# imulki/serenade

Measured on AMD Instinct MI355X. Metric: mel frames/sec converted (UNet ODE + vocoder), 80x1024, higher is better.
Workload: dtype f32

## Files before the change

### include/serenade_hip.h

```cpp
#ifndef SERENADE_HIP_H
#define SERENADE_HIP_H

#include <stdint.h>

#ifdef __cplusplus
extern "C" {
#endif

#define SRN_ABI_VERSION 4
#define SRN_MAX_TAPS 16

enum { SRN_ACT_NONE = 0, SRN_ACT_LEAKY = 1, SRN_ACT_SILU = 2, SRN_ACT_MISH = 3 };
enum { SRN_RES_NONE = 0, SRN_RES_ADD = 1, SRN_RES_AXPY = 2 };
enum {
  SRN_POST_NONE = 0,
  SRN_POST_DIV = 1,
  SRN_POST_TANH = 2,
  SRN_POST_RELU = 3,
  SRN_POST_LEAKY = 4,
  SRN_POST_GELU = 5
};
enum {
  SRN_PREC_FP32 = 0,
  SRN_PREC_BF16X3 = 1,
// ... 69 lines not shown

int srn_resblock_tail(const float* c2, const float* gn_partials, const float* gamma, const float* beta,
                      const int32_t* lens, const float* r, const float* scale, const float* shift, int64_t ld_ss,
                      float* y, int B, int T, int C, int groups, float gn_eps, float ln_eps, int valid_stats,
                      void* stream);

int srn_resblock_tail_ln(const float* c2, const float* gn_partials, const float* gamma, const float* beta,
                         const int32_t* lens, const float* r, const float* scale, const float* shift, int64_t ld_ss,
                         float* y, int B, int T, int C, int groups, float gn_eps, float ln_eps, int valid_stats,
                         const float* ln2_gamma, const float* ln2_beta, float* y2, float ln2_eps, void* stream);

int srn_layernorm(const float* x, const float* gamma, const float* beta, float* y, int64_t rows, int C, float eps,
                  void* stream);

int srn_softmax_rows(float* s, const int32_t* lens, int Z, int n_head, int L, int ld, void* stream);

int srn_sinusoidal_emb(const float* t, float* out, int n, int dim, int ld, float scale, void* stream);

int srn_copy_channels(const float* src, int64_t src_bs, int ld_src, int sc0, float* dst, int64_t dst_bs, int ld_dst,
                      int dc0, int B, int T, int C, void* stream);

int srn_scatter_rows(const float* src, int64_t src_bs, int ld_src, float* dst, int64_t dst_bs, int ld_dst, int dc0,
                     const int32_t* row_off, const int32_t* n_rows, int B, int T, int C, void* stream);

int srn_transpose_ct(const float* src, float* dst, int B, int R, int Cc, int64_t src_bs, int ld_src, int64_t dst_bs,
                     int ld_dst, void* stream);
#define SRN_TR_LIST_MAX 40
typedef struct SrnTransposeList {
  int32_t n;
  int32_t pad_;
// ... 210 lines not shown
```

### serenade_amd/_lib.py

```python
import ctypes
import os
from ctypes import POINTER, c_char_p, c_double, c_float, c_int, c_int32, c_int64, c_void_p

_HERE = os.path.dirname(os.path.abspath(__file__))
LIB_PATH = os.environ.get("SERENADE_AMD_LIB") or os.path.join(_HERE, "libserenade_hip.so")

SRN_MAX_TAPS = 16
ACT_NONE, ACT_LEAKY, ACT_SILU, ACT_MISH = 0, 1, 2, 3
RES_NONE, RES_ADD, RES_AXPY = 0, 1, 2
POST_NONE, POST_DIV, POST_TANH, POST_RELU, POST_LEAKY, POST_GELU = 0, 1, 2, 3, 4, 5
PREC_FP32, PREC_BF16X3, PREC_BF16X6 = 0, 1, 2
ROUTE_AUTO, ROUTE_TILED, ROUTE_HALO, ROUTE_GENERIC, ROUTE_STRIP, ROUTE_FAST_FP32 = 0, 1, 2, 3, 4, 5
FAMILY_GENERIC, FAMILY_F32, FAMILY_FAST, FAMILY_HALO, FAMILY_STRIP = 0, 1, 2, 3, 4
RESUNIT_ROUTE_SHARED = 1
TN_ROUTE_GENERAL = 1


class SrnConvParams(ctypes.Structure):
    _fields_ = [
        ("n_batch", c_int32), ("n_head", c_int32), ("T_in", c_int32), ("T_out", c_int32),
        ("C_in", c_int32), ("C_in0", c_int32), ("C_w", c_int32), ("N", c_int32), ("N_out", c_int32),
        ("n_taps", c_int32), ("tap_off", c_int32 * SRN_MAX_TAPS), ("in_stride", c_int32),
        ("pad_reflect", c_int32), ("w_nmajor", c_int32), ("pro_act", c_int32), ("pro_slope", c_float),
        ("alpha", c_float), ("beta", c_float), ("geglu", c_int32), ("res_mode", c_int32), ("post", c_int32), ("post_div", c_float),
# ... 78 lines not shown
_SIGS = {
    "srn_abi_version": (c_int, []),
    "srn_last_error": (c_char_p, []),
    "srn_conv_gemm": (c_int, [POINTER(SrnConvParams), _P]),
    "srn_conv_gemm_workspace_bytes": (c_int64, [POINTER(SrnConvParams)]),
    "srn_conv_gemm_route": (c_int, [POINTER(SrnConvParams), POINTER(c_int32)]),
    "srn_hifigan_resunit": (c_int, [POINTER(SrnResUnitParams), _P]),
    "srn_gn_mish_apply": (c_int, [_P, _P, _P, _P, _P, c_int64, _P, _P, c_int, c_int, c_int, c_int, c_float, c_int, _P]),
    "srn_resblock_tail": (c_int, [_P, _P, _P, _P, _P, _P, _P, _P, c_int64, _P, c_int, c_int, c_int, c_int,
                                  c_float, c_float, c_int, _P]),
    "srn_resblock_tail_ln": (c_int, [_P, _P, _P, _P, _P, _P, _P, _P, c_int64, _P, c_int, c_int, c_int, c_int,
                                     c_float, c_float, c_int, _P, _P, _P, c_float, _P]),
    "srn_scatter_rows": (c_int, [_P, c_int64, c_int, _P, c_int64, c_int, c_int, _P, _P, c_int, c_int, c_int, _P]),
    "srn_layernorm": (c_int, [_P, _P, _P, _P, c_int64, c_int, c_float, _P]),
    "srn_softmax_rows": (c_int, [_P, _P, c_int, c_int, c_int, c_int, _P]),
    "srn_sinusoidal_emb": (c_int, [_P, _P, c_int, c_int, c_int, c_float, _P]),
    "srn_copy_channels": (c_int, [_P, c_int64, c_int, c_int, _P, c_int64, c_int, c_int, c_int, c_int, c_int, _P]),
    "srn_transpose_ct": (c_int, [_P, _P, c_int, c_int, c_int, c_int64, c_int, c_int64, c_int, _P]),
    "srn_transpose_multi": (c_int, [POINTER(SrnTransposeList), _P]),
    "srn_weight_norm_fwd": (c_int, [_P, _P, _P, _P, _P, c_int, c_int, c_int, _P]),
    "srn_weight_norm_bwd": (c_int, [_P, _P, _P, _P, _P, _P, c_int, c_int, c_int, _P]),
    "srn_renorm": (c_int, [_P, _P, _P, _P, _P, _P, c_int64, c_int, _P]),
    "srn_out_conv_tanh": (c_int, [_P, _P, _P, _P, c_int, c_int, c_int, c_int, c_float, _P]),
    "srn_pd_gather": (c_int, [_P, _P, _P, c_int, c_int, c_int, c_float, c_float, _P]),
    "srn_pad_signal": (c_int, [_P, _P, c_int, c_int, c_int, c_int, c_int, _P]),
    "srn_logmel": (c_int, [_P, _P, _P, c_int64, c_int, c_int, c_int, c_float, c_int, _P]),
    "srn_loudness": (c_int, [_P, _P, _P, _P, c_int, c_int, c_int, c_int, c_float, c_float, c_float, _P]),
    "srn_gru_recur_last": (c_int, [_P, _P, _P, _P, c_int, c_int, c_int, _P]),
    "srn_style_token_attention_kv": (c_int, [_P] * 8 + [c_int] * 5 + [_P]),
    "srn_rowln_fwd": (c_int, [_P, _P, c_int64, _P, c_int64, _P, c_int, c_int, c_int, c_float, _P]),
# ... 79 lines not shown
```

### serenade_amd/csrc/norm_act.hip

```cpp
#include "common.h"
#include "conv_common.h"

namespace {

__device__ __forceinline__ void group_stats(const float* __restrict__ partials, int b, int T, int C, int groups,
                                            float eps, float* s_mean, float* s_rstd, int n_rows) {
  const int gn_mt = (T + 31) / 32;
  const int gn_nt = C / 32;
  const int nt_per_g = (C / groups) / 32;
  const int wave = threadIdx.x >> 6, lane = threadIdx.x & 63;
  const float* base = partials + (int64_t)b * gn_mt * gn_nt * 2;
  const int per_g = gn_mt * nt_per_g;
  for (int g = wave; g < groups; g += 4) {
    double s1 = 0.0, s2 = 0.0;
    for (int e = lane; e < per_g; e += 64) {
      const int mt = e / nt_per_g;
      const int nt = g * nt_per_g + (e - mt * nt_per_g);
      const float2 v = *reinterpret_cast<const float2*>(base + ((int64_t)mt * gn_nt + nt) * 2);
      s1 += (double)v.x;
      s2 += (double)v.y;
    }
    s1 = wave_sum_d(s1);
    s2 = wave_sum_d(s2);
    if (lane == 0) {
      const double cnt = (double)max(n_rows, 1) * (double)(C / groups);
      const double mean = s1 / cnt;
      double var = s2 / cnt - mean * mean;
      if (var < 0.0) var = 0.0;
      s_mean[g] = (float)mean;
      s_rstd[g] = (float)(1.0 / sqrt(var + (double)eps));
    }
  }
  __syncthreads();
}

constexpr int GN_ROWS = 8;
constexpr int SMALL_GRID = 512;
constexpr int GN_PRE = 4;

__global__ __launch_bounds__(256) void gn_mish_apply_kernel(const float* __restrict__ x,
                                                            const float* __restrict__ partials,
                                                            const float* __restrict__ gamma,
                                                            const float* __restrict__ beta,
                                                            const float* __restrict__ time_bias,
                                                            const int32_t* __restrict__ lens, float* __restrict__ y,
                                                            int T, int C, int groups, float eps, int64_t tb_bs,
                                                            int valid_stats, int rows_per_wg) {
  __shared__ float s_mean[64], s_rstd[64];
  const int b = blockIdx.y;
  const int r0 = blockIdx.x * rows_per_wg;
  if (time_bias) time_bias += (int64_t)b * tb_bs;
  const int len = lens ? min(lens[b], T) : T;
  const int c4n = C / 4;
  const int cpg = C / groups;
  const int rows = min(rows_per_wg, T - r0);
// ... 35 lines not shown
  };
#pragma unroll
  for (int k = 0; k < GN_PRE; ++k)
    if ((int)threadIdx.x + 256 * k < total) one(threadIdx.x + 256 * k, pre[k]);
  for (int idx = threadIdx.x + 256 * GN_PRE; idx < total; idx += 256) {
    const int r = idx / c4n;
    float4 v = make_float4(0.f, 0.f, 0.f, 0.f);
    if (r0 + r < len) v = *reinterpret_cast<const float4*>(x + base + (int64_t)r * C + (idx - r * c4n) * 4);
    one(idx, v);
  }
}

constexpr int TAIL_ROWS = 8;
constexpr int MAXV = 4;

__global__ __launch_bounds__(256) void resblock_tail_kernel(
    const float* __restrict__ c2, const float* __restrict__ partials, const float* __restrict__ gamma,
    const float* __restrict__ beta, const int32_t* __restrict__ lens, const float* __restrict__ rres,
    const float* __restrict__ scale, const float* __restrict__ shift, int64_t ld_ss, float* __restrict__ y, int T,
    int C, int groups, float gn_eps, float ln_eps, int valid_stats, const float* __restrict__ ln2_gamma,
    const float* __restrict__ ln2_beta, float* __restrict__ y2, float ln2_eps, int rows_per_wg) {
  __shared__ float s_mean[64], s_rstd[64];
  const int b = blockIdx.y;
  const int r0 = blockIdx.x * rows_per_wg;
  const int len = lens ? min(lens[b], T) : T;
  const int wave = threadIdx.x >> 6, lane = threadIdx.x & 63;
  const int c4n = C / 4;
  const int cpg = C / groups;
  const float inv_c = 1.0f / (float)C;
  const int r_end = min(r0 + rows_per_wg, T);
  float4 xin[MAXV], rin[MAXV];
// ... 88 lines not shown
          const int c = c4 * 4;
          const float4 ga = *reinterpret_cast<const float4*>(ln2_gamma + c);
          const float4 be = *reinterpret_cast<const float4*>(ln2_beta + c);
          float4 o;
          o.x = (v[i].x - mean2) * rstd2 * ga.x + be.x;
          o.y = (v[i].y - mean2) * rstd2 * ga.y + be.y;
          o.z = (v[i].z - mean2) * rstd2 * ga.z + be.z;
          o.w = (v[i].w - mean2) * rstd2 * ga.w + be.w;
          *reinterpret_cast<float4*>(y2 + row + c) = o;
        }
      }
    }
  }
}

__global__ __launch_bounds__(256) void layernorm_kernel(const float* __restrict__ x, const float* __restrict__ gamma,
                                                        const float* __restrict__ beta, float* __restrict__ y,
                                                        int64_t rows, int C, float eps) {
  const int wave = threadIdx.x >> 6, lane = threadIdx.x & 63;
  const int c4n = C / 4;
  const float inv_c = 1.0f / (float)C;
  for (int64_t r = (int64_t)blockIdx.x * 4 + wave; r < rows; r += (int64_t)gridDim.x * 4) {
    const int64_t row = r * C;
    float4 v[MAXV];
    float sum = 0.f;
#pragma unroll
    for (int i = 0; i < MAXV; ++i) {
      const int c4 = lane + 64 * i;
      v[i] = make_float4(0.f, 0.f, 0.f, 0.f);
      if (c4 < c4n) {
        v[i] = *reinterpret_cast<const float4*>(x + row + c4 * 4);
// ... 17 lines not shown
        const int c = c4 * 4;
        const float4 ga = *reinterpret_cast<const float4*>(gamma + c);
        const float4 be = *reinterpret_cast<const float4*>(beta + c);
        float4 o;
        o.x = (v[i].x - mean) * rstd * ga.x + be.x;
        o.y = (v[i].y - mean) * rstd * ga.y + be.y;
        o.z = (v[i].z - mean) * rstd * ga.z + be.z;
        o.w = (v[i].w - mean) * rstd * ga.w + be.w;
        *reinterpret_cast<float4*>(y + row + c) = o;
      }
    }
  }
}

template <int NV>
__global__ __launch_bounds__(256) void softmax_rows_kernel(float* __restrict__ s, const int32_t* __restrict__ lens,
                                                           int64_t n_rows, int n_head, int L, int ld) {
  const int wave = threadIdx.x >> 6, lane = threadIdx.x & 63;
  const int64_t r = (int64_t)blockIdx.x * 4 + wave;
  if (r >= n_rows) return;
  const int z = (int)(r / L);
  int len = L;
  if (lens) len = min(lens[z / n_head], L);
  float* row = s + r * ld;
  const int ld4 = ld / 4;
  float4 v[NV];
  float mx = -INFINITY;
#pragma unroll
  for (int i = 0; i < NV; ++i) {
    const int c4 = lane + 64 * i;
    v[i] = make_float4(-INFINITY, -INFINITY, -INFINITY, -INFINITY);
// ... 19 lines not shown
      sum += (v[i].x + v[i].y) + (v[i].z + v[i].w);
    }
  }
  sum = wave_sum(sum);
#pragma unroll
  for (int i = 0; i < NV; ++i) {
    const int c4 = lane + 64 * i;
    if (c4 < ld4) {
      float4 o;
      o.x = v[i].x / sum;
      o.y = v[i].y / sum;
      o.z = v[i].z / sum;
      o.w = v[i].w / sum;
      *reinterpret_cast<float4*>(row + c4 * 4) = o;
    }
  }
}

__global__ void sinusoidal_emb_kernel(const float* __restrict__ t, float* __restrict__ out, int n, int dim,
                                      int ld, float scale) {
  const int half = dim / 2;
  const int idx = blockIdx.x * blockDim.x + threadIdx.x;
  if (idx >= n * half) return;
  const int i = idx / half, k = idx - i * half;
  const float emb = logf(10000.0f) / (float)(half - 1);
  const float f = expf((float)k * -emb);
  const float arg = scale * t[i] * f;
  out[(int64_t)i * ld + k] = sinf(arg);
  out[(int64_t)i * ld + half + k] = cosf(arg);
}
// ... 140 lines not shown
  float acc = bias[0];
  for (int j = 0; j < K; ++j) {
    const int ti = t + j - (K - 1) / 2;
    if (ti < 0 || ti >= T) continue;
    for (int c = 0; c < C; ++c) {
      float v = xb[(int64_t)ti * C + c];
      v = v > 0.f ? v : v * slope;
      acc = fmaf(v, w[j * C + c], acc);
    }
  }
  y[(int64_t)b * T + t] = tanhf(acc);
}

}

extern "C" int srn_gn_mish_apply(const float* x, const float* gn_partials, const float* gamma, const float* beta,
                                 const float* time_bias, int64_t time_bias_bs, const int32_t* lens, float* y, int B,
                                 int T, int C, int groups, float eps, int valid_stats, void* stream) {
  SRN_CHECK_ARG(x && gn_partials && gamma && beta && y, "gn_mish_apply: null pointer");
  SRN_CHECK_ARG(!valid_stats || lens, "gn_mish_apply: valid_stats needs lens");
  SRN_CHECK_ARG(B > 0 && T > 0 && C > 0 && groups > 0 && groups <= 64 && C % groups == 0 && (C / groups) % 32 == 0,
                "gn_mish_apply: need (C / groups) %% 32 == 0 (C=%d groups=%d)", C, groups);
  const int rows_per_wg = (int64_t)B * ((T + GN_ROWS - 1) / GN_ROWS) < SMALL_GRID ? GN_ROWS / 2 : GN_ROWS;
  dim3 grid((T + rows_per_wg - 1) / rows_per_wg, B);
  hipLaunchKernelGGL(gn_mish_apply_kernel, grid, dim3(256), 0, (hipStream_t)stream, x, gn_partials, gamma, beta,
                     time_bias, lens, y, T, C, groups, eps, time_bias_bs, valid_stats, rows_per_wg);
  SRN_CHECK_LAUNCH();
  return 0;
}

extern "C" int srn_resblock_tail(const float* c2, const float* gn_partials, const float* gamma, const float* beta,
                                 const int32_t* lens, const float* r, const float* scale, const float* shift,
                                 int64_t ld_ss, float* y, int B, int T, int C, int groups, float gn_eps,
                                 float ln_eps, int valid_stats, void* stream) {
  SRN_CHECK_ARG(c2 && gn_partials && gamma && beta && r && scale && shift && y, "resblock_tail: null pointer");
  SRN_CHECK_ARG(!valid_stats || lens, "resblock_tail: valid_stats needs lens");
  SRN_CHECK_ARG(B > 0 && T > 0 && C > 0 && C % 4 == 0 && C <= 256 * MAXV, "resblock_tail: C=%d unsupported", C);
  SRN_CHECK_ARG(groups > 0 && groups <= 64 && C % groups == 0 && (C / groups) % 32 == 0,
                "resblock_tail: need (C / groups) %% 32 == 0");
  const int rows_per_wg = (int64_t)B * ((T + TAIL_ROWS - 1) / TAIL_ROWS) < SMALL_GRID ? TAIL_ROWS / 2 : TAIL_ROWS;
  dim3 grid((T + rows_per_wg - 1) / rows_per_wg, B);
  hipLaunchKernelGGL(resblock_tail_kernel, grid, dim3(256), 0, (hipStream_t)stream, c2, gn_partials, gamma, beta,
                     lens, r, scale, shift, ld_ss, y, T, C, groups, gn_eps, ln_eps, valid_stats, nullptr, nullptr,
                     nullptr, 0.f, rows_per_wg);
  SRN_CHECK_LAUNCH();
  return 0;
}

extern "C" int srn_resblock_tail_ln(const float* c2, const float* gn_partials, const float* gamma, const float* beta,
                                    const int32_t* lens, const float* r, const float* scale, const float* shift,
                                    int64_t ld_ss, float* y, int B, int T, int C, int groups, float gn_eps,
                                    float ln_eps, int valid_stats, const float* ln2_gamma, const float* ln2_beta,
                                    float* y2, float ln2_eps, void* stream) {
  SRN_CHECK_ARG(c2 && gn_partials && gamma && beta && r && scale && shift && y && ln2_gamma && ln2_beta && y2,
                "resblock_tail_ln: null pointer");
  SRN_CHECK_ARG(!valid_stats || lens, "resblock_tail_ln: valid_stats needs lens");
  SRN_CHECK_ARG(B > 0 && T > 0 && C > 0 && C % 4 == 0 && C <= 256 * MAXV, "resblock_tail_ln: C=%d unsupported", C);
  SRN_CHECK_ARG(groups > 0 && groups <= 64 && C % groups == 0 && (C / groups) % 32 == 0,
                "resblock_tail_ln: need (C / groups) %% 32 == 0");
  const int rows_per_wg = (int64_t)B * ((T + TAIL_ROWS - 1) / TAIL_ROWS) < SMALL_GRID ? TAIL_ROWS / 2 : TAIL_ROWS;
  dim3 grid((T + rows_per_wg - 1) / rows_per_wg, B);
  hipLaunchKernelGGL(resblock_tail_kernel, grid, dim3(256), 0, (hipStream_t)stream, c2, gn_partials, gamma, beta,
                     lens, r, scale, shift, ld_ss, y, T, C, groups, gn_eps, ln_eps, valid_stats, ln2_gamma, ln2_beta,
                     y2, ln2_eps, rows_per_wg);
  SRN_CHECK_LAUNCH();
  return 0;
}

extern "C" int srn_layernorm(const float* x, const float* gamma, const float* beta, float* y, int64_t rows, int C,
                             float eps, void* stream) {
  SRN_CHECK_ARG(x && gamma && beta && y, "layernorm: null pointer");
  SRN_CHECK_ARG(rows > 0 && C > 0 && C % 4 == 0 && C <= 256 * MAXV, "layernorm: C=%d unsupported", C);
  int64_t blocks = (rows + 3) / 4;
  if (blocks > 65536) blocks = 65536;
  hipLaunchKernelGGL(layernorm_kernel, dim3((unsigned)blocks), dim3(256), 0, (hipStream_t)stream, x, gamma, beta, y,
                     rows, C, eps);
  SRN_CHECK_LAUNCH();
  return 0;
}

extern "C" int srn_softmax_rows(float* s, const int32_t* lens, int Z, int n_head, int L, int ld, void* stream) {
  SRN_CHECK_ARG(s != nullptr && Z > 0 && n_head > 0 && L > 0 && ld >= L && ld % 4 == 0, "softmax_rows: bad args");
  const int64_t rows = (int64_t)Z * L;
  const unsigned blocks = (unsigned)((rows + 3) / 4);
  const int nv = (ld / 4 + 63) / 64;
  hipStream_t st = (hipStream_t)stream;
  if (nv <= 2) hipLaunchKernelGGL(softmax_rows_kernel<2>, dim3(blocks), dim3(256), 0, st, s, lens, rows, n_head, L, ld);
  else if (nv <= 4) hipLaunchKernelGGL(softmax_rows_kernel<4>, dim3(blocks), dim3(256), 0, st, s, lens, rows, n_head, L, ld);
  else if (nv <= 8) hipLaunchKernelGGL(softmax_rows_kernel<8>, dim3(blocks), dim3(256), 0, st, s, lens, rows, n_head, L, ld);
  else if (nv <= 12) hipLaunchKernelGGL(softmax_rows_kernel<12>, dim3(blocks), dim3(256), 0, st, s, lens, rows, n_head, L, ld);
  else if (nv <= 20) hipLaunchKernelGGL(softmax_rows_kernel<20>, dim3(blocks), dim3(256), 0, st, s, lens, rows, n_head, L, ld);
  else if (nv <= 36) hipLaunchKernelGGL(softmax_rows_kernel<36>, dim3(blocks), dim3(256), 0, st, s, lens, rows, n_head, L, ld);
  else {
    srn_set_error("softmax_rows: L=%d too long (max 9216)", L);
    return -1;
  }
  SRN_CHECK_LAUNCH();
  return 0;
}

extern "C" int srn_sinusoidal_emb(const float* t, float* out, int n, int dim, int ld, float scale, void* stream) {
  SRN_CHECK_ARG(t && out && n > 0 && dim > 2 && dim % 2 == 0 && ld >= dim, "sinusoidal_emb: bad args");
  const int total = n * (dim / 2);
  hipLaunchKernelGGL(sinusoidal_emb_kernel, dim3((total + 255) / 256), dim3(256), 0, (hipStream_t)stream, t, out, n,
                     dim, ld, scale);
  SRN_CHECK_LAUNCH();
  return 0;
}

extern "C" int srn_copy_channels(const float* src, int64_t src_bs, int ld_src, int sc0, float* dst, int64_t dst_bs,
                                 int ld_dst, int dc0, int B, int T, int C, void* stream) {
// ... 120 lines not shown
```

Measured before the change: 61660.

## Make row-wise norm/softmax kernels persistent with double-buffered buffer loads

```diff
diff --git a/include/serenade_hip.h b/include/serenade_hip.h
--- a/include/serenade_hip.h
+++ b/include/serenade_hip.h
@@ -107,6 +107,21 @@
                   void* stream);
 
 int srn_softmax_rows(float* s, const int32_t* lens, int Z, int n_head, int L, int ld, void* stream);
+
+int srn_gn_mish_apply_r4(const float* x, const float* gn_partials, const float* gamma, const float* beta,
+                         const float* time_bias, int64_t time_bias_bs, const int32_t* lens, float* y, int B, int T,
+                         int C, int groups, float eps, int valid_stats, void* stream);
+int srn_resblock_tail_r4(const float* c2, const float* gn_partials, const float* gamma, const float* beta,
+                         const int32_t* lens, const float* r, const float* scale, const float* shift, int64_t ld_ss,
+                         float* y, int B, int T, int C, int groups, float gn_eps, float ln_eps, int valid_stats,
+                         void* stream);
+int srn_resblock_tail_ln_r4(const float* c2, const float* gn_partials, const float* gamma, const float* beta,
+                            const int32_t* lens, const float* r, const float* scale, const float* shift, int64_t ld_ss,
+                            float* y, int B, int T, int C, int groups, float gn_eps, float ln_eps, int valid_stats,
+                            const float* ln2_gamma, const float* ln2_beta, float* y2, float ln2_eps, void* stream);
+int srn_layernorm_r4(const float* x, const float* gamma, const float* beta, float* y, int64_t rows, int C, float eps,
+                     void* stream);
+int srn_softmax_rows_r4(float* s, const int32_t* lens, int Z, int n_head, int L, int ld, void* stream);
 
 int srn_sinusoidal_emb(const float* t, float* out, int n, int dim, int ld, float scale, void* stream);
 
diff --git a/serenade_amd/_lib.py b/serenade_amd/_lib.py
--- a/serenade_amd/_lib.py
+++ b/serenade_amd/_lib.py
@@ -116,6 +116,13 @@
     "srn_scatter_rows": (c_int, [_P, c_int64, c_int, _P, c_int64, c_int, c_int, _P, _P, c_int, c_int, c_int, _P]),
     "srn_layernorm": (c_int, [_P, _P, _P, _P, c_int64, c_int, c_float, _P]),
     "srn_softmax_rows": (c_int, [_P, _P, c_int, c_int, c_int, c_int, _P]),
+    "srn_gn_mish_apply_r4": (c_int, [_P, _P, _P, _P, _P, c_int64, _P, _P, c_int, c_int, c_int, c_int, c_float, c_int, _P]),
+    "srn_resblock_tail_r4": (c_int, [_P, _P, _P, _P, _P, _P, _P, _P, c_int64, _P, c_int, c_int, c_int, c_int,
+                                     c_float, c_float, c_int, _P]),
+    "srn_resblock_tail_ln_r4": (c_int, [_P, _P, _P, _P, _P, _P, _P, _P, c_int64, _P, c_int, c_int, c_int, c_int,
+                                        c_float, c_float, c_int, _P, _P, _P, c_float, _P]),
+    "srn_layernorm_r4": (c_int, [_P, _P, _P, _P, c_int64, c_int, c_float, _P]),
+    "srn_softmax_rows_r4": (c_int, [_P, _P, c_int, c_int, c_int, c_int, _P]),
     "srn_sinusoidal_emb": (c_int, [_P, _P, c_int, c_int, c_int, c_float, _P]),
     "srn_copy_channels": (c_int, [_P, c_int64, c_int, c_int, _P, c_int64, c_int, c_int, c_int, c_int, c_int, _P]),
     "srn_transpose_ct": (c_int, [_P, _P, c_int, c_int, c_int, c_int64, c_int, c_int64, c_int, _P]),
diff --git a/serenade_amd/csrc/norm_act.hip b/serenade_amd/csrc/norm_act.hip
--- a/serenade_amd/csrc/norm_act.hip
+++ b/serenade_amd/csrc/norm_act.hip
@@ -1,5 +1,7 @@
 #include "common.h"
 #include "conv_common.h"
+
+#include <algorithm>
 
 namespace {
 
@@ -38,7 +40,7 @@
 constexpr int SMALL_GRID = 512;
 constexpr int GN_PRE = 4;
 
-__global__ __launch_bounds__(256) void gn_mish_apply_kernel(const float* __restrict__ x,
+__global__ __launch_bounds__(256) void gn_mish_apply_r4_kernel(const float* __restrict__ x,
                                                             const float* __restrict__ partials,
                                                             const float* __restrict__ gamma,
                                                             const float* __restrict__ beta,
@@ -104,7 +106,7 @@
 constexpr int TAIL_ROWS = 8;
 constexpr int MAXV = 4;
 
-__global__ __launch_bounds__(256) void resblock_tail_kernel(
+__global__ __launch_bounds__(256) void resblock_tail_r4_kernel(
     const float* __restrict__ c2, const float* __restrict__ partials, const float* __restrict__ gamma,
     const float* __restrict__ beta, const int32_t* __restrict__ lens, const float* __restrict__ rres,
     const float* __restrict__ scale, const float* __restrict__ shift, int64_t ld_ss, float* __restrict__ y, int T,
@@ -223,7 +225,7 @@
   }
 }
 
-__global__ __launch_bounds__(256) void layernorm_kernel(const float* __restrict__ x, const float* __restrict__ gamma,
+__global__ __launch_bounds__(256) void layernorm_r4_kernel(const float* __restrict__ x, const float* __restrict__ gamma,
                                                         const float* __restrict__ beta, float* __restrict__ y,
                                                         int64_t rows, int C, float eps) {
   const int wave = threadIdx.x >> 6, lane = threadIdx.x & 63;
@@ -271,7 +273,7 @@
 }
 
 template <int NV>
-__global__ __launch_bounds__(256) void softmax_rows_kernel(float* __restrict__ s, const int32_t* __restrict__ lens,
+__global__ __launch_bounds__(256) void softmax_rows_r4_kernel(float* __restrict__ s, const int32_t* __restrict__ lens,
                                                            int64_t n_rows, int n_head, int L, int ld) {
   const int wave = threadIdx.x >> 6, lane = threadIdx.x & 63;
   const int64_t r = (int64_t)blockIdx.x * 4 + wave;
@@ -321,6 +323,399 @@
       o.w = v[i].w / sum;
       *reinterpret_cast<float4*>(row + c4 * 4) = o;
     }
+  }
+}
+
+constexpr int ROW_WGS_PER_CU = 4;
+
+typedef unsigned rw_u32x4 __attribute__((ext_vector_type(4)));
+
+__device__ __forceinline__ __amdgpu_buffer_rsrc_t row_rsrc(const float* row, int bytes) {
+  return __builtin_amdgcn_make_buffer_rsrc(const_cast<float*>(row), 0, bytes, 0x00020000);
+}
+__device__ __forceinline__ float4 row_ld(__amdgpu_buffer_rsrc_t rs, int off) {
+  return __builtin_bit_cast(float4, __builtin_amdgcn_raw_buffer_load_b128(rs, off, 0, 0));
+}
+__device__ __forceinline__ void row_st(const float4 v, __amdgpu_buffer_rsrc_t rs, int off) {
+  __builtin_amdgcn_raw_buffer_store_b128(__builtin_bit_cast(rw_u32x4, v), rs, off, 0, 0);
+}
+
+__device__ __forceinline__ void gn_worker_rows(int T, int rpw, int& t_begin, int& t_end) {
+  t_begin = blockIdx.x * 4 * rpw;
+  t_end = min(t_begin + 4 * rpw, T);
+}
+
+template <int NV>
+__global__ __launch_bounds__(256) void gn_mish_apply_kernel(const float* __restrict__ x,
+                                                            const float* __restrict__ partials,
+                                                            const float* __restrict__ gamma,
+                                                            const float* __restrict__ beta,
+                                                            const float* __restrict__ time_bias,
+                                                            const int32_t* __restrict__ lens, float* __restrict__ y,
+                                                            int T, int C, int groups, float eps, int64_t tb_bs,
+                                                            int valid_stats, int rpw) {
+  __shared__ float s_mean[64], s_rstd[64];
+  const int b = blockIdx.y;
+  const int wave = __builtin_amdgcn_readfirstlane(threadIdx.x >> 6), lane = threadIdx.x & 63;
+  int t_begin, t_end;
+  gn_worker_rows(T, rpw, t_begin, t_end);
+  const int len = lens ? min(lens[b], T) : T;
+  const int c4n = C / 4;
+  const int cpg = C / groups;
+  const float* xb = x + (int64_t)b * T * C;
+  float* yb = y + (int64_t)b * T * C;
+  auto fetch = [&](float4 (&v)[NV], const int t) {
+    if (t >= len) return;
+    const __amdgpu_buffer_rsrc_t rs = row_rsrc(xb + (int64_t)t * C, C * 4);
+#pragma unroll
+    for (int i = 0; i < NV; ++i)
+      if (lane + 64 * i < c4n) v[i] = row_ld(rs, (lane + 64 * i) * 16);
+  };
+  float4 va[NV], vb[NV];
+  int t = t_begin + wave;
+  if (t < t_end) fetch(va, t);
+  group_stats(partials, b, T, C, groups, eps, s_mean, s_rstd, valid_stats ? len : T);
+  float4 ga[NV], be[NV], tb[NV];
+  float m[NV], rsd[NV];
+#pragma unroll
+  for (int i = 0; i < NV; ++i) {
+    const int c = (lane + 64 * i) * 4;
+    ga[i] = be[i] = tb[i] = make_float4(0.f, 0.f, 0.f, 0.f);
+    m[i] = rsd[i] = 0.f;
+    if (lane + 64 * i < c4n) {
+      ga[i] = *reinterpret_cast<const float4*>(gamma + c);
+      be[i] = *reinterpret_cast<const float4*>(beta + c);
+      if (time_bias) tb[i] = *reinterpret_cast<const float4*>(time_bias + (int64_t)b * tb_bs + c);
+      m[i] = s_mean[c / cpg];
+      rsd[i] = s_rstd[c / cpg];
+    }
+  }
+  auto finish = [&](const float4 (&v)[NV], const int t) {
+    const __amdgpu_buffer_rsrc_t rs = row_rsrc(yb + (int64_t)t * C, C * 4);
+    const bool valid = t < len;
+#pragma unroll
+    for (int i = 0; i < NV; ++i) {
+      if (lane + 64 * i < c4n) {
+        float4 o = make_float4(0.f, 0.f, 0.f, 0.f);
+        if (valid) {
+          o.x = srn_mish((v[i].x - m[i]) * rsd[i] * ga[i].x + be[i].x);
+          o.y = srn_mish((v[i].y - m[i]) * rsd[i] * ga[i].y + be[i].y);
+          o.z = srn_mish((v[i].z - m[i]) * rsd[i] * ga[i].z + be[i].z);
+          o.w = srn_mish((v[i].w - m[i]) * rsd[i] * ga[i].w + be[i].w);
+          if (time_bias) {
+            o.x += tb[i].x;
+            o.y += tb[i].y;
+            o.z += tb[i].z;
+            o.w += tb[i].w;
+          }
+        }
+        row_st(o, rs, (lane + 64 * i) * 16);
+      }
+    }
+  };
+  while (t < t_end) {
+    if (t + 4 < t_end) fetch(vb, t + 4);
+    finish(va, t);
+    t += 4;
+    if (t >= t_end) break;
+    if (t + 4 < t_end) fetch(va, t + 4);
+    finish(vb, t);
+    t += 4;
+  }
+}
+
+template <int NV>
+__global__ __launch_bounds__(256) void resblock_tail_kernel(
+    const float* __restrict__ c2, const float* __restrict__ partials, const float* __restrict__ gamma,
+    const float* __restrict__ beta, const int32_t* __restrict__ lens, const float* __restrict__ rres,
+    const float* __restrict__ scale, const float* __restrict__ shift, int64_t ld_ss, float* __restrict__ y, int T,
+    int C, int groups, float gn_eps, float ln_eps, int valid_stats, const float* __restrict__ ln2_gamma,
+    const float* __restrict__ ln2_beta, float* __restrict__ y2, float ln2_eps, int rpw) {
+  __shared__ float s_mean[64], s_rstd[64];
+  const int b = blockIdx.y;
+  const int wave = __builtin_amdgcn_readfirstlane(threadIdx.x >> 6), lane = threadIdx.x & 63;
+  int t_begin, t_end;
+  gn_worker_rows(T, rpw, t_begin, t_end);
+  const int len = lens ? min(lens[b], T) : T;
+  const int c4n = C / 4;
+  const int cpg = C / groups;
+  const float inv_c = 1.0f / (float)C;
+  const int64_t base = (int64_t)b * T * C;
+  struct Row {
+    float4 x[NV], r[NV];
+  };
+  auto fetch = [&](Row& a, const int t) {
+    const __amdgpu_buffer_rsrc_t rr = row_rsrc(rres + base + (int64_t)t * C, C * 4);
+    const __amdgpu_buffer_rsrc_t rx = row_rsrc(c2 + base + (int64_t)t * C, C * 4);
+#pragma unroll
+    for (int i = 0; i < NV; ++i) {
+      a.x[i] = a.r[i] = make_float4(0.f, 0.f, 0.f, 0.f);
+      if (lane + 64 * i < c4n) {
+        a.r[i] = row_ld(rr, (lane + 64 * i) * 16);
+        if (t < len) a.x[i] = row_ld(rx, (lane + 64 * i) * 16);
+      }
+    }
+  };
+  Row ra, rb;
+  int t = t_begin + wave;
+  if (t < t_end) fetch(ra, t);
+  group_stats(partials, b, T, C, groups, gn_eps, s_mean, s_rstd, valid_stats ? len : T);
+  float4 ga[NV], be[NV], sc[NV], sh[NV], lg[NV], lb[NV];
+  float m[NV], rsd[NV];
+#pragma unroll
+  for (int i = 0; i < NV; ++i) {
+    const int c = (lane + 64 * i) * 4;
+    ga[i] = be[i] = sc[i] = sh[i] = lg[i] = lb[i] = make_float4(0.f, 0.f, 0.f, 0.f);
+    m[i] = rsd[i] = 0.f;
+    if (lane + 64 * i < c4n) {
+      ga[i] = *reinterpret_cast<const float4*>(gamma + c);
+      be[i] = *reinterpret_cast<const float4*>(beta + c);
+      sc[i] = *reinterpret_cast<const float4*>(scale + (int64_t)b * ld_ss + c);
+      sh[i] = *reinterpret_cast<const float4*>(shift + (int64_t)b * ld_ss + c);
+      if (y2 != nullptr) {
+        lg[i] = *reinterpret_cast<const float4*>(ln2_gamma + c);
+        lb[i] = *reinterpret_cast<const float4*>(ln2_beta + c);
+      }
+      m[i] = s_mean[c / cpg];
+      rsd[i] = s_rstd[c / cpg];
+    }
+  }
+  auto finish = [&](const Row& a, const int t) {
+    const int64_t row = base + (int64_t)t * C;
+    const bool valid = t < len;
+    float4 v[NV];
+    float sum = 0.f;
+#pragma unroll
+    for (int i = 0; i < NV; ++i) {
+      v[i] = make_float4(0.f, 0.f, 0.f, 0.f);
+      if (lane + 64 * i < c4n) {
+        const float4 rr = a.r[i];
+        float4 o = make_float4(0.f, 0.f, 0.f, 0.f);
+        if (valid) {
+          const float4 xx = a.x[i];
+          o.x = srn_mish((xx.x - m[i]) * rsd[i] * ga[i].x + be[i].x);
+          o.y = srn_mish((xx.y - m[i]) * rsd[i] * ga[i].y + be[i].y);
+          o.z = srn_mish((xx.z - m[i]) * rsd[i] * ga[i].z + be[i].z);
+          o.w = srn_mish((xx.w - m[i]) * rsd[i] * ga[i].w + be[i].w);
+        }
+        v[i] = make_float4(o.x + rr.x, o.y + rr.y, o.z + rr.z, o.w + rr.w);
+        sum += (v[i].x + v[i].y) + (v[i].z + v[i].w);
+      }
+    }
+    const float mean = wave_sum(sum) * inv_c;
+    float sq = 0.f;
+#pragma unroll
+    for (int i = 0; i < NV; ++i) {
+      if (lane + 64 * i < c4n) {
+        const float dx = v[i].x - mean, dy = v[i].y - mean, dz = v[i].z - mean, dw = v[i].w - mean;
+        sq += (dx * dx + dy * dy) + (dz * dz + dw * dw);
+      }
+    }
+    const float stdv = sqrtf(wave_sum(sq) * inv_c + ln_eps);
+    const __amdgpu_buffer_rsrc_t ry = row_rsrc(y + row, C * 4);
+#pragma unroll
+    for (int i = 0; i < NV; ++i) {
+      if (lane + 64 * i < c4n) {
+        float4 o;
+        o.x = (v[i].x - mean) / stdv * sc[i].x + sh[i].x;
+        o.y = (v[i].y - mean) / stdv * sc[i].y + sh[i].y;
+        o.z = (v[i].z - mean) / stdv * sc[i].z + sh[i].z;
+        o.w = (v[i].w - mean) / stdv * sc[i].w + sh[i].w;
+        row_st(o, ry, (lane + 64 * i) * 16);
+        v[i] = o;
+      }
+    }
+    if (y2 != nullptr) {
+      float sum2 = 0.f;
+#pragma unroll
+      for (int i = 0; i < NV; ++i)
+        if (lane + 64 * i < c4n) sum2 += (v[i].x + v[i].y) + (v[i].z + v[i].w);
+      const float mean2 = wave_sum(sum2) * inv_c;
+      float sq2 = 0.f;
+#pragma unroll
+      for (int i = 0; i < NV; ++i) {
+        if (lane + 64 * i < c4n) {
+          const float dx = v[i].x - mean2, dy = v[i].y - mean2, dz = v[i].z - mean2, dw = v[i].w - mean2;
+          sq2 += (dx * dx + dy * dy) + (dz * dz + dw * dw);
+        }
+      }
+      const float rstd2 = 1.0f / sqrtf(wave_sum(sq2) * inv_c + ln2_eps);
+      const __amdgpu_buffer_rsrc_t ry2 = row_rsrc(y2 + row, C * 4);
+#pragma unroll
+      for (int i = 0; i < NV; ++i) {
+        if (lane + 64 * i < c4n) {
+          float4 o;
+          o.x = (v[i].x - mean2) * rstd2 * lg[i].x + lb[i].x;
+          o.y = (v[i].y - mean2) * rstd2 * lg[i].y + lb[i].y;
+          o.z = (v[i].z - mean2) * rstd2 * lg[i].z + lb[i].z;
+          o.w = (v[i].w - mean2) * rstd2 * lg[i].w + lb[i].w;
+          row_st(o, ry2, (lane + 64 * i) * 16);
+        }
+      }
+    }
+  };
+  while (t < t_end) {
+    if (t + 4 < t_end) fetch(rb, t + 4);
+    finish(ra, t);
+    t += 4;
+    if (t >= t_end) break;
+    if (t + 4 < t_end) fetch(ra, t + 4);
+    finish(rb, t);
+    t += 4;
+  }
+}
+
+template <int NV>
+__global__ __launch_bounds__(256) void layernorm_kernel(const float* __restrict__ x, const float* __restrict__ gamma,
+                                                        const float* __restrict__ beta, float* __restrict__ y,
+                                                        int64_t rows, int C, float eps) {
+  const int lane = threadIdx.x & 63;
+  const int64_t stride = (int64_t)gridDim.x * 4;
+  int64_t r = (int64_t)blockIdx.x * 4 + __builtin_amdgcn_readfirstlane(threadIdx.x >> 6);
+  if (r >= rows) return;
+  const int c4n = C / 4;
+  const float inv_c = 1.0f / (float)C;
+  auto fetch = [&](float4 (&v)[NV], const int64_t rr) {
+    const __amdgpu_buffer_rsrc_t rs = row_rsrc(x + rr * C, C * 4);
+#pragma unroll
+    for (int i = 0; i < NV; ++i)
+      if (lane + 64 * i < c4n) v[i] = row_ld(rs, (lane + 64 * i) * 16);
+  };
+  float4 va[NV], vb[NV];
+  fetch(va, r);
+  float4 ga[NV], be[NV];
+#pragma unroll
+  for (int i = 0; i < NV; ++i) {
+    ga[i] = be[i] = make_float4(0.f, 0.f, 0.f, 0.f);
+    if (lane + 64 * i < c4n) {
+      ga[i] = *reinterpret_cast<const float4*>(gamma + (lane + 64 * i) * 4);
+      be[i] = *reinterpret_cast<const float4*>(beta + (lane + 64 * i) * 4);
+    }
+  }
+  auto finish = [&](const float4 (&v)[NV], const int64_t rr) {
+    float sum = 0.f;
+#pragma unroll
+    for (int i = 0; i < NV; ++i)
+      if (lane + 64 * i < c4n) sum += (v[i].x + v[i].y) + (v[i].z + v[i].w);
+    const float mean = wave_sum(sum) * inv_c;
+    float sq = 0.f;
+#pragma unroll
+    for (int i = 0; i < NV; ++i) {
+      if (lane + 64 * i < c4n) {
+        const float dx = v[i].x - mean, dy = v[i].y - mean, dz = v[i].z - mean, dw = v[i].w - mean;
+        sq += (dx * dx + dy * dy) + (dz * dz + dw * dw);
+      }
+    }
+    const float rstd = 1.0f / sqrtf(wave_sum(sq) * inv_c + eps);
+    const __amdgpu_buffer_rsrc_t rs = row_rsrc(y + rr * C, C * 4);
+#pragma unroll
+    for (int i = 0; i < NV; ++i) {
+      if (lane + 64 * i < c4n) {
+        float4 o;
+        o.x = (v[i].x - mean) * rstd * ga[i].x + be[i].x;
+        o.y = (v[i].y - mean) * rstd * ga[i].y + be[i].y;
+        o.z = (v[i].z - mean) * rstd * ga[i].z + be[i].z;
+        o.w = (v[i].w - mean) * rstd * ga[i].w + be[i].w;
+        row_st(o, rs, (lane + 64 * i) * 16);
+      }
+    }
+  };
+  for (;;) {
+    if (r + stride < rows) fetch(vb, r + stride);
+    finish(va, r);
+    r += stride;
+    if (r >= rows) return;
+    if (r + stride < rows) fetch(va, r + stride);
+    finish(vb, r);
+    r += stride;
+    if (r >= rows) return;
+  }
+}
+
+template <int NV>
+struct SmRow {
+  float4 v[NV];
+  int len;
+};
+
+template <int NV, bool AHEAD>
+__global__ __launch_bounds__(256) void softmax_rows_kernel(float* __restrict__ s, const int32_t* __restrict__ lens,
+                                                           int n_rows, int n_head, int L, int ld) {
+  const int lane = threadIdx.x & 63;
+  const int stride = gridDim.x * 4;
+  int r = blockIdx.x * 4 + __builtin_amdgcn_readfirstlane(threadIdx.x >> 6);
+  if (r >= n_rows) return;
+  const int ld4 = ld / 4;
+  auto fetch = [&](SmRow<NV>& a, const int rr) {
+    const __amdgpu_buffer_rsrc_t rs = row_rsrc(s + (int64_t)rr * ld, ld * 4);
+#pragma unroll
+    for (int i = 0; i < NV; ++i)
+      if (lane + 64 * i < ld4) a.v[i] = row_ld(rs, (lane + 64 * i) * 16);
+    a.len = lens ? min(lens[rr / L / n_head], L) : L;
+  };
+  auto finish = [&](const SmRow<NV>& a, const int rr) {
+    const int len = a.len;
+    float4 v[NV];
+    float mx = -INFINITY;
+#pragma unroll
+    for (int i = 0; i < NV; ++i) {
+      const int c4 = lane + 64 * i;
+      v[i] = make_float4(-INFINITY, -INFINITY, -INFINITY, -INFINITY);
+      if (c4 < ld4) {
+        const float4 t = a.v[i];
+        const int c = c4 * 4;
+        if (c + 0 < len) v[i].x = t.x;
+        if (c + 1 < len) v[i].y = t.y;
+        if (c + 2 < len) v[i].z = t.z;
+        if (c + 3 < len) v[i].w = t.w;
+        mx = fmaxf(mx, fmaxf(fmaxf(v[i].x, v[i].y), fmaxf(v[i].z, v[i].w)));
+      }
+    }
+    mx = wave_max(mx);
+    float sum = 0.f;
+#pragma unroll
+    for (int i = 0; i < NV; ++i) {
+      if (lane + 64 * i < ld4) {
+        v[i].x = expf(v[i].x - mx);
+        v[i].y = expf(v[i].y - mx);
+        v[i].z = expf(v[i].z - mx);
+        v[i].w = expf(v[i].w - mx);
+        sum += (v[i].x + v[i].y) + (v[i].z + v[i].w);
+      }
+    }
+    sum = wave_sum(sum);
+    const __amdgpu_buffer_rsrc_t rs = row_rsrc(s + (int64_t)rr * ld, ld * 4);
+#pragma unroll
+    for (int i = 0; i < NV; ++i) {
+      const int c4 = lane + 64 * i;
+      if (c4 < ld4) {
+        float4 o;
+        o.x = v[i].x / sum;
+        o.y = v[i].y / sum;
+        o.z = v[i].z / sum;
+        o.w = v[i].w / sum;
+        row_st(o, rs, c4 * 16);
+      }
+    }
+  };
+  SmRow<NV> ra, rb;
+  fetch(ra, r);
+  for (;;) {
+    if (!AHEAD) {
+      finish(ra, r);
+      r += stride;
+      if (r >= n_rows) return;
+      fetch(ra, r);
+      continue;
+    }
+    if (r + stride < n_rows) fetch(rb, r + stride);
+    finish(ra, r);
+    r += stride;
+    if (r >= n_rows) return;
+    if (r + stride < n_rows) fetch(ra, r + stride);
+    finish(rb, r);
+    r += stride;
+    if (r >= n_rows) return;
   }
 }
 
@@ -491,7 +886,7 @@
 
 }
 
-extern "C" int srn_gn_mish_apply(const float* x, const float* gn_partials, const float* gamma, const float* beta,
+extern "C" int srn_gn_mish_apply_r4(const float* x, const float* gn_partials, const float* gamma, const float* beta,
                                  const float* time_bias, int64_t time_bias_bs, const int32_t* lens, float* y, int B,
                                  int T, int C, int groups, float eps, int valid_stats, void* stream) {
   SRN_CHECK_ARG(x && gn_partials && gamma && beta && y, "gn_mish_apply: null pointer");
@@ -500,13 +895,13 @@
                 "gn_mish_apply: need (C / groups) %% 32 == 0 (C=%d groups=%d)", C, groups);
   const int rows_per_wg = (int64_t)B * ((T + GN_ROWS - 1) / GN_ROWS) < SMALL_GRID ? GN_ROWS / 2 : GN_ROWS;
   dim3 grid((T + rows_per_wg - 1) / rows_per_wg, B);
-  hipLaunchKernelGGL(gn_mish_apply_kernel, grid, dim3(256), 0, (hipStream_t)stream, x, gn_partials, gamma, beta,
+  hipLaunchKernelGGL(gn_mish_apply_r4_kernel, grid, dim3(256), 0, (hipStream_t)stream, x, gn_partials, gamma, beta,
                      time_bias, lens, y, T, C, groups, eps, time_bias_bs, valid_stats, rows_per_wg);
   SRN_CHECK_LAUNCH();
   return 0;
 }
 
-extern "C" int srn_resblock_tail(const float* c2, const float* gn_partials, const float* gamma, const float* beta,
+extern "C" int srn_resblock_tail_r4(const float* c2, const float* gn_partials, const float* gamma, const float* beta,
                                  const int32_t* lens, const float* r, const float* scale, const float* shift,
                                  int64_t ld_ss, float* y, int B, int T, int C, int groups, float gn_eps,
                                  float ln_eps, int valid_stats, void* stream) {
@@ -517,14 +912,14 @@
                 "resblock_tail: need (C / groups) %% 32 == 0");
   const int rows_per_wg = (int64_t)B * ((T + TAIL_ROWS - 1) / TAIL_ROWS) < SMALL_GRID ? TAIL_ROWS / 2 : TAIL_ROWS;
   dim3 grid((T + rows_per_wg - 1) / rows_per_wg, B);
-  hipLaunchKernelGGL(resblock_tail_kernel, grid, dim3(256), 0, (hipStream_t)stream, c2, gn_partials, gamma, beta,
+  hipLaunchKernelGGL(resblock_tail_r4_kernel, grid, dim3(256), 0, (hipStream_t)stream, c2, gn_partials, gamma, beta,
                      lens, r, scale, shift, ld_ss, y, T, C, groups, gn_eps, ln_eps, valid_stats, nullptr, nullptr,
                      nullptr, 0.f, rows_per_wg);
   SRN_CHECK_LAUNCH();
   return 0;
 }
 
-extern "C" int srn_resblock_tail_ln(const float* c2, const float* gn_partials, const float* gamma, const float* beta,
+extern "C" int srn_resblock_tail_ln_r4(const float* c2, const float* gn_partials, const float* gamma, const float* beta,
                                     const int32_t* lens, const float* r, const float* scale, const float* shift,
                                     int64_t ld_ss, float* y, int B, int T, int C, int groups, float gn_eps,
                                     float ln_eps, int valid_stats, const float* ln2_gamma, const float* ln2_beta,
@@ -537,41 +932,193 @@
                 "resblock_tail_ln: need (C / groups) %% 32 == 0");
   const int rows_per_wg = (int64_t)B * ((T + TAIL_ROWS - 1) / TAIL_ROWS) < SMALL_GRID ? TAIL_ROWS / 2 : TAIL_ROWS;
   dim3 grid((T + rows_per_wg - 1) / rows_per_wg, B);
-  hipLaunchKernelGGL(resblock_tail_kernel, grid, dim3(256), 0, (hipStream_t)stream, c2, gn_partials, gamma, beta,
+  hipLaunchKernelGGL(resblock_tail_r4_kernel, grid, dim3(256), 0, (hipStream_t)stream, c2, gn_partials, gamma, beta,
                      lens, r, scale, shift, ld_ss, y, T, C, groups, gn_eps, ln_eps, valid_stats, ln2_gamma, ln2_beta,
                      y2, ln2_eps, rows_per_wg);
   SRN_CHECK_LAUNCH();
   return 0;
 }
 
-extern "C" int srn_layernorm(const float* x, const float* gamma, const float* beta, float* y, int64_t rows, int C,
+extern "C" int srn_layernorm_r4(const float* x, const float* gamma, const float* beta, float* y, int64_t rows, int C,
                              float eps, void* stream) {
   SRN_CHECK_ARG(x && gamma && beta && y, "layernorm: null pointer");
   SRN_CHECK_ARG(rows > 0 && C > 0 && C % 4 == 0 && C <= 256 * MAXV, "layernorm: C=%d unsupported", C);
   int64_t blocks = (rows + 3) / 4;
   if (blocks > 65536) blocks = 65536;
-  hipLaunchKernelGGL(layernorm_kernel, dim3((unsigned)blocks), dim3(256), 0, (hipStream_t)stream, x, gamma, beta, y,
+  hipLaunchKernelGGL(layernorm_r4_kernel, dim3((unsigned)blocks), dim3(256), 0, (hipStream_t)stream, x, gamma, beta, y,
                      rows, C, eps);
   SRN_CHECK_LAUNCH();
   return 0;
 }
 
-extern "C" int srn_softmax_rows(float* s, const int32_t* lens, int Z, int n_head, int L, int ld, void* stream) {
+extern "C" int srn_softmax_rows_r4(float* s, const int32_t* lens, int Z, int n_head, int L, int ld, void* stream) {
   SRN_CHECK_ARG(s != nullptr && Z > 0 && n_head > 0 && L > 0 && ld >= L && ld % 4 == 0, "softmax_rows: bad args");
   const int64_t rows = (int64_t)Z * L;
   const unsigned blocks = (unsigned)((rows + 3) / 4);
   const int nv = (ld / 4 + 63) / 64;
   hipStream_t st = (hipStream_t)stream;
-  if (nv <= 2) hipLaunchKernelGGL(softmax_rows_kernel<2>, dim3(blocks), dim3(256), 0, st, s, lens, rows, n_head, L, ld);
-  else if (nv <= 4) hipLaunchKernelGGL(softmax_rows_kernel<4>, dim3(blocks), dim3(256), 0, st, s, lens, rows, n_head, L, ld);
-  else if (nv <= 8) hipLaunchKernelGGL(softmax_rows_kernel<8>, dim3(blocks), dim3(256), 0, st, s, lens, rows, n_head, L, ld);
-  else if (nv <= 12) hipLaunchKernelGGL(softmax_rows_kernel<12>, dim3(blocks), dim3(256), 0, st, s, lens, rows, n_head, L, ld);
-  else if (nv <= 20) hipLaunchKernelGGL(softmax_rows_kernel<20>, dim3(blocks), dim3(256), 0, st, s, lens, rows, n_head, L, ld);
-  else if (nv <= 36) hipLaunchKernelGGL(softmax_rows_kernel<36>, dim3(blocks), dim3(256), 0, st, s, lens, rows, n_head, L, ld);
+  if (nv <= 2) hipLaunchKernelGGL(softmax_rows_r4_kernel<2>, dim3(blocks), dim3(256), 0, st, s, lens, rows, n_head, L, ld);
+  else if (nv <= 4) hipLaunchKernelGGL(softmax_rows_r4_kernel<4>, dim3(blocks), dim3(256), 0, st, s, lens, rows, n_head, L, ld);
+  else if (nv <= 8) hipLaunchKernelGGL(softmax_rows_r4_kernel<8>, dim3(blocks), dim3(256), 0, st, s, lens, rows, n_head, L, ld);
+  else if (nv <= 12) hipLaunchKernelGGL(softmax_rows_r4_kernel<12>, dim3(blocks), dim3(256), 0, st, s, lens, rows, n_head, L, ld);
+  else if (nv <= 20) hipLaunchKernelGGL(softmax_rows_r4_kernel<20>, dim3(blocks), dim3(256), 0, st, s, lens, rows, n_head, L, ld);
+  else if (nv <= 36) hipLaunchKernelGGL(softmax_rows_r4_kernel<36>, dim3(blocks), dim3(256), 0, st, s, lens, rows, n_head, L, ld);
   else {
     srn_set_error("softmax_rows: L=%d too long (max 9216)", L);
     return -1;
   }
+  SRN_CHECK_LAUNCH();
+  return 0;
+}
+
+static int rows_cu_count() {
+  static std::atomic<int> cached[64];
+  int dev = 0;
+  if (hipGetDevice(&dev) != hipSuccess || dev < 0 || dev >= 64) dev = 0;
+  int n = cached[dev].load(std::memory_order_relaxed);
+  if (n <= 0) {
+    if (hipDeviceGetAttribute(&n, hipDeviceAttributeMultiprocessorCount, dev) != hipSuccess || n <= 0) n = 1;
+    cached[dev].store(n, std::memory_order_relaxed);
+  }
+  return n;
+}
+
+template <auto K>
+static int row_wgs_per_cu() {
+  static std::atomic<int> cached{0};
+  int n = cached.load(std::memory_order_relaxed);
+  if (n <= 0) {
+    if (hipOccupancyMaxActiveBlocksPerMultiprocessor(&n, K, 256, 0) != hipSuccess || n <= 0) n = 1;
+    n = std::min(n, ROW_WGS_PER_CU);
+    cached.store(n, std::memory_order_relaxed);
+  }
+  return n;
+}
+
+template <auto K>
+static unsigned row_blocks(int64_t quads) {
+  return (unsigned)std::max<int64_t>(1, std::min<int64_t>(quads, (int64_t)rows_cu_count() * row_wgs_per_cu<K>()));
+}
+
+template <auto K>
+static dim3 gn_rows_grid(int B, int T, int& rpw) {
+  const int want = max(1, (rows_cu_count() * row_wgs_per_cu<K>() + B - 1) / B);
+  rpw = max(1, (T + 4 * want - 1) / (4 * want));
+  return dim3((T + 4 * rpw - 1) / (4 * rpw), B);
+}
+
+extern "C" int srn_gn_mish_apply(const float* x, const float* gn_partials, const float* gamma, const float* beta,
+                                 const float* time_bias, int64_t time_bias_bs, const int32_t* lens, float* y, int B,
+                                 int T, int C, int groups, float eps, int valid_stats, void* stream) {
+  SRN_CHECK_ARG(x && gn_partials && gamma && beta && y, "gn_mish_apply: null pointer");
+  SRN_CHECK_ARG(!valid_stats || lens, "gn_mish_apply: valid_stats needs lens");
+  SRN_CHECK_ARG(B > 0 && T > 0 && C > 0 && groups > 0 && groups <= 64 && C % groups == 0 && (C / groups) % 32 == 0,
+                "gn_mish_apply: need (C / groups) %% 32 == 0 (C=%d groups=%d)", C, groups);
+  if (C > 256 * MAXV)
+    return srn_gn_mish_apply_r4(x, gn_partials, gamma, beta, time_bias, time_bias_bs, lens, y, B, T, C, groups, eps,
+                                valid_stats, stream);
+  int rpw;
+  hipStream_t st = (hipStream_t)stream;
+#define SRN_GN_LAUNCH(NV)                                                                                        \
+  do {                                                                                                           \
+    const dim3 grid = gn_rows_grid<gn_mish_apply_kernel<NV>>(B, T, rpw);                                         \
+    hipLaunchKernelGGL(gn_mish_apply_kernel<NV>, grid, dim3(256), 0, st, x, gn_partials, gamma, beta, time_bias, \
+                       lens, y, T, C, groups, eps, time_bias_bs, valid_stats, rpw);                              \
+  } while (0)
+  if (C <= 256) SRN_GN_LAUNCH(1);
+  else if (C <= 512) SRN_GN_LAUNCH(2);
+  else SRN_GN_LAUNCH(4);
+#undef SRN_GN_LAUNCH
+  SRN_CHECK_LAUNCH();
+  return 0;
+}
+
+static int resblock_tail_launch(const float* c2, const float* gn_partials, const float* gamma, const float* beta,
+                                const int32_t* lens, const float* r, const float* scale, const float* shift,
+                                int64_t ld_ss, float* y, int B, int T, int C, int groups, float gn_eps, float ln_eps,
+                                int valid_stats, const float* ln2_gamma, const float* ln2_beta, float* y2,
+                                float ln2_eps, void* stream) {
+  int rpw;
+  hipStream_t st = (hipStream_t)stream;
+#define SRN_TAIL_LAUNCH(NV)                                                                                      \
+  do {                                                                                                           \
+    const dim3 grid = gn_rows_grid<resblock_tail_kernel<NV>>(B, T, rpw);                                         \
+    hipLaunchKernelGGL(resblock_tail_kernel<NV>, grid, dim3(256), 0, st, c2, gn_partials, gamma, beta, lens, r,   \
+                       scale, shift, ld_ss, y, T, C, groups, gn_eps, ln_eps, valid_stats, ln2_gamma, ln2_beta, y2, \
+                       ln2_eps, rpw);                                                                            \
+  } while (0)
+  if (C <= 512) SRN_TAIL_LAUNCH(2);
+  else SRN_TAIL_LAUNCH(4);
+#undef SRN_TAIL_LAUNCH
+  SRN_CHECK_LAUNCH();
+  return 0;
+}
+
+extern "C" int srn_resblock_tail(const float* c2, const float* gn_partials, const float* gamma, const float* beta,
+                                 const int32_t* lens, const float* r, const float* scale, const float* shift,
+                                 int64_t ld_ss, float* y, int B, int T, int C, int groups, float gn_eps,
+                                 float ln_eps, int valid_stats, void* stream) {
+  SRN_CHECK_ARG(c2 && gn_partials && gamma && beta && r && scale && shift && y, "resblock_tail: null pointer");
+  SRN_CHECK_ARG(!valid_stats || lens, "resblock_tail: valid_stats needs lens");
+  SRN_CHECK_ARG(B > 0 && T > 0 && C > 0 && C % 4 == 0 && C <= 256 * MAXV, "resblock_tail: C=%d unsupported", C);
+  SRN_CHECK_ARG(groups > 0 && groups <= 64 && C % groups == 0 && (C / groups) % 32 == 0,
+                "resblock_tail: need (C / groups) %% 32 == 0");
+  return resblock_tail_launch(c2, gn_partials, gamma, beta, lens, r, scale, shift, ld_ss, y, B, T, C, groups, gn_eps,
+                              ln_eps, valid_stats, nullptr, nullptr, nullptr, 0.f, stream);
+}
+
+extern "C" int srn_resblock_tail_ln(const float* c2, const float* gn_partials, const float* gamma, const float* beta,
+                                    const int32_t* lens, const float* r, const float* scale, const float* shift,
+                                    int64_t ld_ss, float* y, int B, int T, int C, int groups, float gn_eps,
+                                    float ln_eps, int valid_stats, const float* ln2_gamma, const float* ln2_beta,
+                                    float* y2, float ln2_eps, void* stream) {
+  SRN_CHECK_ARG(c2 && gn_partials && gamma && beta && r && scale && shift && y && ln2_gamma && ln2_beta && y2,
+                "resblock_tail_ln: null pointer");
+  SRN_CHECK_ARG(!valid_stats || lens, "resblock_tail_ln: valid_stats needs lens");
+  SRN_CHECK_ARG(B > 0 && T > 0 && C > 0 && C % 4 == 0 && C <= 256 * MAXV, "resblock_tail_ln: C=%d unsupported", C);
+  SRN_CHECK_ARG(groups > 0 && groups <= 64 && C % groups == 0 && (C / groups) % 32 == 0,
+                "resblock_tail_ln: need (C / groups) %% 32 == 0");
+  return resblock_tail_launch(c2, gn_partials, gamma, beta, lens, r, scale, shift, ld_ss, y, B, T, C, groups, gn_eps,
+                              ln_eps, valid_stats, ln2_gamma, ln2_beta, y2, ln2_eps, stream);
+}
+
+extern "C" int srn_layernorm(const float* x, const float* gamma, const float* beta, float* y, int64_t rows, int C,
+                             float eps, void* stream) {
+  SRN_CHECK_ARG(x && gamma && beta && y, "layernorm: null pointer");
+  SRN_CHECK_ARG(rows > 0 && C > 0 && C % 4 == 0 && C <= 256 * MAXV, "layernorm: C=%d unsupported", C);
+  hipStream_t st = (hipStream_t)stream;
+#define SRN_LN_LAUNCH(NV)                                                                                          \
+  hipLaunchKernelGGL(layernorm_kernel<NV>, dim3(row_blocks<layernorm_kernel<NV>>((rows + 3) / 4)), dim3(256), 0, st, x, \
+                     gamma, beta, y, rows, C, eps)
+  if (C <= 512) SRN_LN_LAUNCH(2);
+  else SRN_LN_LAUNCH(4);
+#undef SRN_LN_LAUNCH
+  SRN_CHECK_LAUNCH();
+  return 0;
+}
+
+extern "C" int srn_softmax_rows(float* s, const int32_t* lens, int Z, int n_head, int L, int ld, void* stream) {
+  SRN_CHECK_ARG(s != nullptr && Z > 0 && n_head > 0 && L > 0 && ld >= L && ld % 4 == 0, "softmax_rows: bad args");
+  SRN_CHECK_ARG((int64_t)Z * L < (1ll << 31), "softmax_rows: Z * L = %lld rows too many", (long long)Z * L);
+  const int rows = Z * L;
+  const int nv = (ld / 4 + 63) / 64;
+  hipStream_t st = (hipStream_t)stream;
+#define SRN_SM_LAUNCH(NV, AHEAD)                                                                                     \
+  hipLaunchKernelGGL((softmax_rows_kernel<NV, AHEAD>), dim3(row_blocks<softmax_rows_kernel<NV, AHEAD>>((rows + 3) / 4)), \
+                     dim3(256), 0, st, s, lens, rows, n_head, L, ld)
+  if (nv <= 2) SRN_SM_LAUNCH(2, true);
+  else if (nv <= 3) SRN_SM_LAUNCH(3, true);
+  else if (nv <= 4) SRN_SM_LAUNCH(4, true);
+  else if (nv <= 5) SRN_SM_LAUNCH(5, true);
+  else if (nv <= 8) SRN_SM_LAUNCH(8, true);
+  else if (nv <= 12) SRN_SM_LAUNCH(12, true);
+  else if (nv <= 20) SRN_SM_LAUNCH(20, false);
+  else if (nv <= 36) SRN_SM_LAUNCH(36, false);
+  else {
+    srn_set_error("softmax_rows: L=%d too long (max 9216)", L);
+    return -1;
+  }
+#undef SRN_SM_LAUNCH
   SRN_CHECK_LAUNCH();
   return 0;
 }
```

New measurement: 61830, median of 6. About the same (+0.3%).
